# cpuimage/minSDTF

Hardware: AMD Instinct MI355X
Metric: 512x512 images/sec (whole node), SD1.5 25-step txt2img (higher is better)
Workload: dtype bf16; 1 GPU; SD1.5 512x512 25-step txt2img, CFG 7.5 + rescale 0.7, batch 1/GPU, UNet+VAE HIP path, random-init weights; global_batch=1, parallelism=batch-shard x1, hipgraph=True, cond_uncond=one fused batch

## Files before the change

minsdtf_amd/csrc/capi.hip:

```cpp
#include <stdarg.h>
#include <string.h>
#include "common.h"

static thread_local char g_err[512] = "";

void msd_set_error(const char* fmt, ...) {
    va_list ap;
    va_start(ap, fmt);
    vsnprintf(g_err, sizeof(g_err), fmt, ap);
    va_end(ap);
}

int msd_conv_gemm_init();
int msd_attention_init();

extern "C" int msd_abi_version(void) { return MSD_ABI_VERSION; }
extern "C" const char* msd_last_error(void) { return g_err; }
extern "C" int msd_init(void) {
    int rc = msd_conv_gemm_init();
    if (rc) return rc;
    return msd_attention_init();
}

void msd_set_gn_impl(int v);
void msd_set_conv_dense(int v);
void msd_set_gn_rows_q(int v);
void msd_set_gn_wide(int v);
void msd_set_gn_cluster(int v);
void msd_set_gn_rows(int v);
void msd_set_gn_xmap(int v);
void msd_set_gn_poll_limit(int v);
void msd_set_attn_qf(int v);
void msd_set_attn_qf4_min(int v);
void msd_set_xattn_nw(int v);
int msd_set_xattn160_mode(int v);
void msd_set_attn_form(int v);
void msd_set_attn_d160_pipe(int v);
extern "C" int msd_set_option(const char* key, int value) {
    if (key && strcmp(key, "gn_rows_q") == 0) {
        if (value < -1 || value > 2) MSD_FAIL(MSD_E_ARG, "set_option: gn_rows_q %d (-1 .. 2)", value);
        msd_set_gn_rows_q(value);
        return MSD_OK;
    }
    if (key && strcmp(key, "conv_dense") == 0) {
        msd_set_conv_dense(value);
        return MSD_OK;
    }
    if (key && strcmp(key, "attn_qf") == 0) {
        if (value < 0 || value > 4 || value == 3) MSD_FAIL(MSD_E_ARG, "set_option: attn_qf takes 0, 1, 2 or 4");
        msd_set_attn_qf(value);
        return MSD_OK;
    }
    if (key && strcmp(key, "attn_qf4_min") == 0) {
        if (value < 128) MSD_FAIL(MSD_E_ARG, "set_option: attn_qf4_min takes a workgroup count >= 128");
        msd_set_attn_qf4_min(value);
        return MSD_OK;
    }
    if (key && strcmp(key, "attn_form") == 0) {
        if (value < 0 || value > 2) MSD_FAIL(MSD_E_ARG, "set_option: attn_form takes 0, 1 or 2");
        msd_set_attn_form(value);
        return MSD_OK;
    }
    if (key && strcmp(key, "attn_d160_pipe") == 0) {
        msd_set_attn_d160_pipe(value ? 1 : 0);
        return MSD_OK;
    }
    if (key && strcmp(key, "xattn160_mode") == 0) {
        if (!msd_set_xattn160_mode(value)) MSD_FAIL(MSD_E_ARG, "set_option: xattn160_mode %d exists in the instrumented build (make stamps) only", value);
        return MSD_OK;
    }
    if (key && strcmp(key, "xattn_nw") == 0) {
        if (value != 0 && value != 4 && value != 8) MSD_FAIL(MSD_E_ARG, "set_option: xattn_nw takes 0, 4 or 8");
        msd_set_xattn_nw(value);
        return MSD_OK;
    }
    if (key && strcmp(key, "gn_wide") == 0) {
        msd_set_gn_wide(value);
        return MSD_OK;
    }
    if (key && strcmp(key, "gn_xmap") == 0) { msd_set_gn_xmap(value); return MSD_OK; }
    if (key && strcmp(key, "gn_rows") == 0) {
        if (value < 0) MSD_FAIL(MSD_E_ARG, "set_option: gn_rows takes a pixel count >= 0, got %d", value);
        msd_set_gn_rows(value);
        return MSD_OK;
    }
    if (key && strcmp(key, "gn_cluster") == 0) {
        if (value != 0 && (value < 64 || value > (1 << 20))) MSD_FAIL(MSD_E_ARG, "set_option: gn_cluster takes 0 or 64 .. 2^20 pixels per part");
        msd_set_gn_cluster(value);
        return MSD_OK;
    }
    if (key && strcmp(key, "gn_poll_limit") == 0) {
        if (value < 1) MSD_FAIL(MSD_E_ARG, "set_option: gn_poll_limit takes a positive count");
        msd_set_gn_poll_limit(value);
        return MSD_OK;
    }
    if (key && strcmp(key, "gn_impl") == 0) {
        msd_set_gn_impl(value);
        return MSD_OK;
    }
    MSD_FAIL(MSD_E_ARG, "set_option: unknown key");
}
```

minsdtf_amd/csrc/conv_rowpanel.hip:

```cpp
#include "conv_common.h"

constexpr int RL_STEPS = 4;
template <int KC, int MI, bool RL = false>
__global__ __launch_bounds__(256) void dense_rowpanel_kernel(const bf16_t* hot_a0, const bf16_t* hot_w, int hot_M, int hot_N, int hot_c0, int hot_tiles_m, int hot_tiles_n,
                                                             uint32_t hot_w_rs, uint32_t hot_w_ks, int wg_cols, int nsplits, uint32_t mg_nsplits, const CGArgs p) {
    constexpr int S = 3, NJ = 2, MP = MI / 2;
    constexpr int BM = 4 * MI * 16;
    constexpr int W_BYTES = KC * 4096;
    static_assert(MI % 2 == 0, "row fragments pair up for the 16-byte stores");
    extern __shared__ __attribute__((aligned(16))) char smem[];
    const uint32_t lds0 = (uint32_t)(size_t)(__attribute__((address_space(3))) char*)smem;
    float* l_bias = reinterpret_cast<float*>(smem + S * W_BYTES);
    float* l_cs = l_bias + wg_cols;

    const int tid = threadIdx.x, lane = tid & 63;
    const int wave = __builtin_amdgcn_readfirstlane(tid >> 6);
    const int r = lane & 15, g = lane >> 4;
    const int tile = xcd_remap(blockIdx.x, hot_tiles_m * hot_tiles_n);
    const int panel = udiv_magic(tile, nsplits, mg_nsplits), ns = tile - panel * nsplits;
    const int m0 = panel * BM + wave * (MI * 16);
    const int n0 = ns * wg_cols;
    const int nsteps = (min(wg_cols, hot_N - n0)) >> 5;

    const int cpos = tid & 7, lrow = tid >> 3;
    const uint32_t wsw = (uint32_t)((cpos ^ ((lrow >> 1) & 7)) * 16);
    const uint32_t lds_wave = lds0 + (uint32_t)(wave * 8) * 128u;
    auto issue_w = [&](int step, int stage) {
        const uint32_t off = (uint32_t)min(n0 + step * 32 + lrow, hot_N - 1) * hot_w_rs + wsw;
        const uint32_t base = __builtin_amdgcn_readfirstlane(lds_wave + (uint32_t)stage * W_BYTES);
#pragma unroll
        for (int kc = 0; kc < KC; ++kc) dma16s(hot_w, off + (uint32_t)kc * hot_w_ks, base + (uint32_t)kc * 4096u);
    };
    if (nsteps > 0) issue_w(0, 0);
    if (nsteps > 1) issue_w(1, 1);

    bf16x8 af[MI][KC * 2];
#pragma unroll
    for (int i = 0; i < MI; ++i) {
        const bf16_t* src = hot_a0 + (size_t)min(m0 + i * 16 + r, hot_M - 1) * hot_c0 + g * 8;
#pragma unroll
        for (int ks = 0; ks < KC * 2; ++ks) af[i][ks] = *reinterpret_cast<const bf16x8*>(src + ks * 32);
    }
    for (int t = tid; t < wg_cols; t += 256) {
        const int n = min(n0 + t, p.N - 1);
        l_bias[t] = p.bias ? p.bias[n] : 0.f;
        l_cs[t] = (!RL && p.ln_in) ? p.ln_colsum[n] : 0.f;
    }
    const int cgo = cg_col(g), cg8 = (g & 1) << 3;
    const int rw = cg_wrow(r);
    int msw[MP], bidx[MI];
#pragma unroll
    for (int ip = 0; ip < MP; ++ip) msw[ip] = m0 + (g < 2 ? 2 * ip : 2 * ip + 1) * 16 + r;
    typedef uint32_t u32x4 __attribute__((ext_vector_type(4)));
    u32x4 rres[RL ? RL_STEPS : 1][MP][NJ];
    if (RL) {
#pragma unroll
        for (int st = 0; st < RL_STEPS; ++st)
#pragma unroll
            for (int ip = 0; ip < MP; ++ip)
#pragma unroll
                for (int j = 0; j < NJ; ++j) {
                    rres[st][ip][j] = (u32x4){0, 0, 0, 0};
                    if (p.residual && st < nsteps)
                        rres[st][ip][j] = *reinterpret_cast<const u32x4*>(p.residual + (size_t)min(msw[ip], p.M - 1) * p.res_ld +
                                                                          min(n0 + st * 32 + j * 16 + cg8, p.N - 8));
                }
    }
    constexpr int LNS = LN_MAX_SLOTS / 4;
    float mean[MI], rstd[MI];
#pragma unroll
    for (int i = 0; i < MI; ++i) { mean[i] = 0.f; rstd[i] = 1.f; }
    if (!RL && p.ln_in) {
        float2 lnp[MI][LNS];
#pragma unroll
        for (int i = 0; i < MI; ++i) {
            const float2* src = reinterpret_cast<const float2*>(p.ln_in) + (size_t)min(m0 + i * 16 + r, p.M - 1) * p.ln_in_slots;
#pragma unroll
            for (int k = 0; k < LNS; ++k) lnp[i][k] = src[min(g + 4 * k, p.ln_in_slots - 1)];
        }
        wait_vmcnt<0>();
#pragma unroll
        for (int i = 0; i < MI; ++i) {
            float s1 = 0.f, s2 = 0.f;
#pragma unroll
            for (int k = 0; k < LNS; ++k)
                if (g + 4 * k < p.ln_in_slots) { s1 += lnp[i][k].x; s2 += lnp[i][k].y; }
            s1 += __shfl_xor(s1, 16); s2 += __shfl_xor(s2, 16);
            s1 += __shfl_xor(s1, 32); s2 += __shfl_xor(s2, 32);
            mean[i] = s1 * p.ln_inv_k;
            rstd[i] = rsqrtf(fmaxf(s2 * p.ln_inv_k - mean[i] * mean[i], 0.f) + p.ln_eps);
        }
    }
    wait_vmcnt<0>();
#pragma unroll
    for (int i = 0; i < MI; ++i)
#pragma unroll
        for (int ks = 0; ks < KC * 2; ++ks) asm volatile("" : "+v"(af[i][ks]));
    if (RL) {
#pragma unroll
        for (int st = 0; st < RL_STEPS; ++st)
#pragma unroll
            for (int ip = 0; ip < MP; ++ip)
#pragma unroll
                for (int j = 0; j < NJ; ++j) asm volatile("" : "+v"(rres[st][ip][j]));
    }
    __syncthreads();

    float lna[MP], lnq[MP];
#pragma unroll
    for (int ip = 0; ip < MP; ++ip) { lna[ip] = 0.f; lnq[ip] = 0.f; }
#pragma unroll
    for (int i = 0; i < MI; ++i) bidx[i] = p.split_mode ? udiv_magic(min(m0 + i * 16 + r, p.M - 1), p.hw_out, p.mg_hw) : 0;
    auto swap8 = [&](const float (&a)[4], const float (&b)[4], float (&v)[8]) {
#pragma unroll
        for (int e = 0; e < 4; ++e) {
            auto sw = __builtin_amdgcn_permlane32_swap(__float_as_uint(a[e]), __float_as_uint(b[e]), false, false);
            v[e] = __uint_as_float(sw[0]);
            v[4 + e] = __uint_as_float(sw[1]);
        }
    };

    int stage = 0;
    for (int step = 0; step < nsteps; ++step) {
        if (step) {
            if (step + 1 < nsteps) wait_vmcnt<KC>();
            else wait_vmcnt<0>();
            __builtin_amdgcn_s_barrier();
        }
        if (step + 2 < nsteps) {
            int st = stage + 2;
            if (st >= S) st -= S;
            issue_w(step + 2, st);
        }
        f32x4 acc[NJ][MI];
#pragma unroll
        for (int j = 0; j < NJ; ++j)
#pragma unroll
            for (int i = 0; i < MI; ++i) acc[j][i] = (f32x4){0.f, 0.f, 0.f, 0.f};
        const char* bW = smem + stage * W_BYTES + rw * 128;
#pragma unroll
        for (int kc = 0; kc < KC; ++kc) {
            bf16x8 wf[2][NJ];
#pragma unroll
            for (int ks = 0; ks < 2; ++ks)
#pragma unroll
                for (int j = 0; j < NJ; ++j)
                    wf[ks][j] = *reinterpret_cast<const bf16x8*>(bW + kc * 4096 + j * 16 * 128 + (((ks * 4 + g) ^ (rw >> 1)) << 4));
#pragma unroll
            for (int ks = 0; ks < 2; ++ks)
#pragma unroll
                for (int j = 0; j < NJ; ++j)
#pragma unroll
                    for (int i = 0; i < MI; ++i)
                        acc[j][i] = __builtin_amdgcn_mfma_f32_16x16x32_bf16(wf[ks][j], af[i][kc * 2 + ks], acc[j][i], 0, 0, 0);
        }
        const int nb = n0 + step * 32;
        float4 bv[NJ], cs[NJ];
#pragma unroll
        for (int j = 0; j < NJ; ++j) {
            bv[j] = *reinterpret_cast<const float4*>(l_bias + step * 32 + j * 16 + cgo);
            cs[j] = *reinterpret_cast<const float4*>(l_cs + step * 32 + j * 16 + cgo);
        }
        if (!RL && p.ln_in) {
#pragma unroll
            for (int i = 0; i < MI; ++i)
#pragma unroll
                for (int j = 0; j < NJ; ++j) {
                    acc[j][i][0] = rstd[i] * (acc[j][i][0] - mean[i] * cs[j].x);
                    acc[j][i][1] = rstd[i] * (acc[j][i][1] - mean[i] * cs[j].y);
                    acc[j][i][2] = rstd[i] * (acc[j][i][2] - mean[i] * cs[j].z);
                    acc[j][i][3] = rstd[i] * (acc[j][i][3] - mean[i] * cs[j].w);
                }
        }
        if constexpr (RL) {
            const float zero = 0.f;
#pragma unroll
            for (int i = 0; i < MI; ++i)
#pragma unroll
                for (int j = 0; j < NJ; ++j) {
                    acc[j][i][0] = (acc[j][i][0] + bv[j].x) + zero; acc[j][i][1] = (acc[j][i][1] + bv[j].y) + zero;
                    acc[j][i][2] = (acc[j][i][2] + bv[j].z) + zero; acc[j][i][3] = (acc[j][i][3] + bv[j].w) + zero;
                }
            if ((step & 1) == 0) {
#pragma unroll
                for (int ip = 0; ip < MP; ++ip) { lna[ip] = 0.f; lnq[ip] = 0.f; }
            }
#pragma unroll
            for (int ip = 0; ip < MP; ++ip)
#pragma unroll
                for (int j = 0; j < NJ; ++j) {
                    float a[4] = {acc[j][2 * ip][0], acc[j][2 * ip][1], acc[j][2 * ip][2], acc[j][2 * ip][3]};
                    float b[4] = {acc[j][2 * ip + 1][0], acc[j][2 * ip + 1][1], acc[j][2 * ip + 1][2], acc[j][2 * ip + 1][3]};
                    float v[8], q[8];
                    swap8(a, b, v);
                    u32x4 rr = rres[0][ip][j];
#pragma unroll
                    for (int st = 1; st < RL_STEPS; ++st) if (step == st) rr = rres[st][ip][j];
                    unpack8(make_uint4(rr.x, rr.y, rr.z, rr.w), q);
#pragma unroll
                    for (int e = 0; e < 8; ++e) v[e] = v[e] + q[e];
                    const uint4 o = pack8(v);
                    const bool ok = msw[ip] < p.M;
                    if (ok) *reinterpret_cast<uint4*>(reinterpret_cast<bf16_t*>(p.out) + (size_t)msw[ip] * p.out_ld + nb + j * 16 + cg8) = o;
                    if (p.ln_out) {
                        unpack8(o, q);
                        float s1 = (ok ? (q[0] + q[1]) + (q[2] + q[3]) : 0.f) + (ok ? (q[4] + q[5]) + (q[6] + q[7]) : 0.f);
                        float s2 = (ok ? (q[0] * q[0] + q[1] * q[1]) + (q[2] * q[2] + q[3] * q[3]) : 0.f) +
                                   (ok ? (q[4] * q[4] + q[5] * q[5]) + (q[6] * q[6] + q[7] * q[7]) : 0.f);
                        auto t1 = __builtin_amdgcn_permlane16_swap(__float_as_uint(s1), __float_as_uint(s1), false, false);
                        auto t2 = __builtin_amdgcn_permlane16_swap(__float_as_uint(s2), __float_as_uint(s2), false, false);
                        lna[ip] += __uint_as_float(t1[0]) + __uint_as_float(t1[1]);
                        lnq[ip] += __uint_as_float(t2[0]) + __uint_as_float(t2[1]);
                    }
                }
            if (p.ln_out && (step & 1) && (g & 1) == 0) {
#pragma unroll
                for (int ip = 0; ip < MP; ++ip)
                    if (msw[ip] < p.M)
                        reinterpret_cast<float2*>(p.ln_out)[(size_t)msw[ip] * p.ln_out_slots + (nb >> 6)] = make_float2(lna[ip], lnq[ip]);
            }
        } else if (p.act == MSD_ACT_GEGLU) {
            auto gl4 = [&](int i, float (&v)[4]) {
                v[0] = geglu_f(acc[0][i][0] + bv[0].x, acc[1][i][0] + bv[1].x);
                v[1] = geglu_f(acc[0][i][1] + bv[0].y, acc[1][i][1] + bv[1].y);
                v[2] = geglu_f(acc[0][i][2] + bv[0].z, acc[1][i][2] + bv[1].z);
                v[3] = geglu_f(acc[0][i][3] + bv[0].w, acc[1][i][3] + bv[1].w);
            };
#pragma unroll
            for (int ip = 0; ip < MP; ++ip) {
                float a[4], b[4], v[8];
                gl4(2 * ip, a);
                gl4(2 * ip + 1, b);
                swap8(a, b, v);
                if (msw[ip] < p.M)
                    *reinterpret_cast<uint4*>(reinterpret_cast<bf16_t*>(p.out) + (size_t)msw[ip] * p.out_ld + (nb >> 1) + cg8) = pack8(v);
            }
        } else {
            const float zero = 0.f;
#pragma unroll
            for (int i = 0; i < MI; ++i)
#pragma unroll
                for (int j = 0; j < NJ; ++j) {
                    acc[j][i][0] = (acc[j][i][0] + bv[j].x) + zero; acc[j][i][1] = (acc[j][i][1] + bv[j].y) + zero;
                    acc[j][i][2] = (acc[j][i][2] + bv[j].z) + zero; acc[j][i][3] = (acc[j][i][3] + bv[j].w) + zero;
                }
#pragma unroll
            for (int j = 0; j < NJ; ++j) {
                const int nbj = nb + j * 16;
                if (p.split_mode == 0 || nbj < p.ns0 + p.ns1) {
#pragma unroll
                    for (int ip = 0; ip < MP; ++ip) {
                        float a[4] = {acc[j][2 * ip][0], acc[j][2 * ip][1], acc[j][2 * ip][2], acc[j][2 * ip][3]};
                        float b[4] = {acc[j][2 * ip + 1][0], acc[j][2 * ip + 1][1], acc[j][2 * ip + 1][2], acc[j][2 * ip + 1][3]};
                        float v[8];
                        swap8(a, b, v);
                        if (p.split_mode == 0) {
#pragma unroll
                            for (int e = 0; e < 8; ++e) v[e] = v[e] + zero;
                        }
                        const int n8 = nbj + cg8;
                        if (msw[ip] >= p.M) continue;
                        bf16_t* dst = (p.split_mode == 0 || n8 < p.ns0) ? reinterpret_cast<bf16_t*>(p.out) + (size_t)msw[ip] * p.out_ld + n8
                                                                         : p.out1 + (size_t)msw[ip] * p.out1_ld + (n8 - p.ns0);
                        *reinterpret_cast<uint4*>(dst) = pack8(v);
                    }
                } else {
                    const int nv = p.N - p.ns0 - p.ns1;
                    const int nn = nbj + cgo - p.ns0 - p.ns1;
#pragma unroll
                    for (int i = 0; i < MI; ++i) {
                        const int m = m0 + i * 16 + r;
                        if (m >= p.M) continue;
                        const int sidx = m - bidx[i] * p.hw_out;
                        const uint32_t ox = pack_bf2(acc[j][i][0], acc[j][i][1]), oy = pack_bf2(acc[j][i][2], acc[j][i][3]);
                        bf16_t* dst = p.out2 + ((size_t)bidx[i] * nv + nn) * p.out2_ld + sidx;
                        dst[0] = (bf16_t)(ox & 0xFFFF);
                        dst[(size_t)p.out2_ld] = (bf16_t)(ox >> 16);
                        dst[(size_t)2 * p.out2_ld] = (bf16_t)(oy & 0xFFFF);
                        dst[(size_t)3 * p.out2_ld] = (bf16_t)(oy >> 16);
                    }
                }
            }
        }
        if (++stage == S) stage = 0;
    }
}

static bool g_rp_attr_done = false;
constexpr int rp_lds(int kc, int wg_cols) { return 3 * kc * 4096 + 2 * wg_cols * 4; }
constexpr int RP_MAX_COLS = 1024;

int msd_conv_rowpanel_init() {
    if (g_rp_attr_done) return MSD_OK;
    hipError_t e = hipFuncSetAttribute(reinterpret_cast<const void*>(&dense_rowpanel_kernel<5, 2>), hipFuncAttributeMaxDynamicSharedMemorySize, rp_lds(5, RP_MAX_COLS));
    if (e == hipSuccess) e = hipFuncSetAttribute(reinterpret_cast<const void*>(&dense_rowpanel_kernel<10, 2>), hipFuncAttributeMaxDynamicSharedMemorySize, rp_lds(10, RP_MAX_COLS));
    if (e == hipSuccess) e = hipFuncSetAttribute(reinterpret_cast<const void*>(&dense_rowpanel_kernel<5, 2, true>), hipFuncAttributeMaxDynamicSharedMemorySize, rp_lds(5, 32 * RL_STEPS));
    if (e == hipSuccess) e = hipFuncSetAttribute(reinterpret_cast<const void*>(&dense_rowpanel_kernel<10, 2, true>), hipFuncAttributeMaxDynamicSharedMemorySize, rp_lds(10, 32 * RL_STEPS));
    if (e != hipSuccess) MSD_FAIL((int)e, "hipFuncSetAttribute(conv_rowpanel): %s", hipGetErrorString(e));
    g_rp_attr_done = true;
    return MSD_OK;
}

bool msd_conv_rowpanel_eligible(const CGArgs& a, int rows, int wg_cols) {
    const bool rl = a.residual || a.ln_out;
    const bool shape = a.ksize == 1 && a.stride == 1 && !a.upsample && a.c1 == 0 && !a.a2 && (a.K == 320 || a.K == 640) && (a.N % 32) == 0 &&
                       !a.rowvec && !a.out_f32 && a.nslices == 1 && a.vec16 &&
                       (a.act == MSD_ACT_NONE || (a.act == MSD_ACT_GEGLU && a.split_mode == 0)) &&
                       (!rl || (a.act == MSD_ACT_NONE && a.split_mode == 0 && !a.ln_in && (a.N % 64) == 0 && (wg_cols % 64) == 0 &&
                                wg_cols <= 32 * RL_STEPS)) &&
                       (long long)a.M * a.c0 * 2 < (1ll << 32) - 4096;
    const bool cfg = rows == 128;
    return shape && cfg && wg_cols >= 32 && wg_cols <= RP_MAX_COLS && (wg_cols % 32) == 0;
}

int msd_conv_rowpanel_launch(CGArgs a, int rows, int wg_cols, hipStream_t stream) {
    int rc = msd_conv_rowpanel_init();
    if (rc) return rc;
    if (wg_cols > a.N) wg_cols = a.N;
    const int panels = (a.M + rows - 1) / rows, nsplits = (a.N + wg_cols - 1) / wg_cols;
    a.tiles_m = panels; a.tiles_n = nsplits;
    const dim3 grid(panels * nsplits);
    const uint32_t mg = udiv_magic_of(nsplits);
    const bool rl = a.residual || a.ln_out;
    if (a.K == 320) {
        if (rl) hipLaunchKernelGGL((dense_rowpanel_kernel<5, 2, true>), grid, dim3(256), rp_lds(5, wg_cols), stream, a.a0, a.w, a.M, a.N, a.c0, a.tiles_m, a.tiles_n, a.w_rs, a.w_ks, wg_cols, nsplits, mg, a);
        else hipLaunchKernelGGL((dense_rowpanel_kernel<5, 2>), grid, dim3(256), rp_lds(5, wg_cols), stream, a.a0, a.w, a.M, a.N, a.c0, a.tiles_m, a.tiles_n, a.w_rs, a.w_ks, wg_cols, nsplits, mg, a);
    } else {
        if (rl) hipLaunchKernelGGL((dense_rowpanel_kernel<10, 2, true>), grid, dim3(256), rp_lds(10, wg_cols), stream, a.a0, a.w, a.M, a.N, a.c0, a.tiles_m, a.tiles_n, a.w_rs, a.w_ks, wg_cols, nsplits, mg, a);
        else hipLaunchKernelGGL((dense_rowpanel_kernel<10, 2>), grid, dim3(256), rp_lds(10, wg_cols), stream, a.a0, a.w, a.M, a.N, a.c0, a.tiles_m, a.tiles_n, a.w_rs, a.w_ks, wg_cols, nsplits, mg, a);
    }
    return MSD_OK;
}
```

Before: 10.39 images/s.

## Software-pipeline K=640 rowpanel GEMM: overlap next tile MFMA with current epilogue

Adds a PIPE variant of the dense rowpanel kernel for K=640 non-residual launches. It double-buffers the accumulators so the MFMA work for the next 32-column step is interleaved with the epilogue of the current step, using sched_group_barrier hints. It also double-buffers the LDS weight fragments across the kc loop and keeps the A fragments in AGPRs. The weight prefetch is moved one step earlier. The variant is on by default and can be switched off through a new rowpanel_pipe option. It risks higher register pressure and a more fragile instruction schedule, and it also adds optional timing-stamp instrumentation under MSD_STAMPS.

```diff
diff --git a/minsdtf_amd/csrc/capi.hip b/minsdtf_amd/csrc/capi.hip
--- a/minsdtf_amd/csrc/capi.hip
+++ b/minsdtf_amd/csrc/capi.hip
@@ -36,6 +36,7 @@
 int msd_set_xattn160_mode(int v);
 void msd_set_attn_form(int v);
 void msd_set_attn_d160_pipe(int v);
+void msd_set_rowpanel_pipe(int v);
 extern "C" int msd_set_option(const char* key, int value) {
     if (key && strcmp(key, "gn_rows_q") == 0) {
         if (value < -1 || value > 2) MSD_FAIL(MSD_E_ARG, "set_option: gn_rows_q %d (-1 .. 2)", value);
@@ -63,6 +64,10 @@
     }
     if (key && strcmp(key, "attn_d160_pipe") == 0) {
         msd_set_attn_d160_pipe(value ? 1 : 0);
+        return MSD_OK;
+    }
+    if (key && strcmp(key, "rowpanel_pipe") == 0) {
+        msd_set_rowpanel_pipe(value ? 1 : 0);
         return MSD_OK;
     }
     if (key && strcmp(key, "xattn160_mode") == 0) {
diff --git a/minsdtf_amd/csrc/conv_rowpanel.hip b/minsdtf_amd/csrc/conv_rowpanel.hip
--- a/minsdtf_amd/csrc/conv_rowpanel.hip
+++ b/minsdtf_amd/csrc/conv_rowpanel.hip
@@ -1,10 +1,65 @@
 #include "conv_common.h"
 
 constexpr int RL_STEPS = 4;
-template <int KC, int MI, bool RL = false>
+
+#ifdef MSD_STAMPS
+extern "C" MSD_API int msd_debug_stamps_rowpanel(unsigned long long* host_out, int count) {
+    return (int)hipMemcpyFromSymbol(host_out, HIP_SYMBOL(g_stamps), sizeof(unsigned long long) * (size_t)count);
+}
+__device__ __forceinline__ unsigned long long rp_now() {
+    unsigned long long t;
+    __builtin_amdgcn_sched_barrier(0);
+    asm volatile("s_memrealtime %0\n\ts_waitcnt lgkmcnt(0)" : "=s"(t)::"memory");
+    __builtin_amdgcn_sched_barrier(0);
+    return t;
+}
+#define RP_STAMP_VARS unsigned long long rp_t = 0, rp_sum[4] = {0, 0, 0, 0}
+#define RP_MARK() rp_t = rp_now()
+#define RP_LAP(i)                                  \
+    do {                                           \
+        const unsigned long long rp_n = rp_now();  \
+        rp_sum[(i) - 8] += rp_n - rp_t;            \
+        rp_t = rp_n;                               \
+    } while (0)
+#define RP_MFMA_RETIRE(x)                                          \
+    do {                                                           \
+        float rp_d;                                                \
+        asm volatile("v_mov_b32 %0, %1" : "=v"(rp_d) : "v"(x));   \
+    } while (0)
+#define RP_STAMP_FLUSH(steps)                                                                                         \
+    do {                                                                                                              \
+        if (threadIdx.x == 0) {                                                                                       \
+            unsigned long long* rp_o = g_stamps + (((size_t)blockIdx.y * gridDim.x + blockIdx.x) & 8191) * 16;        \
+            rp_o[8] = rp_sum[0]; rp_o[9] = rp_sum[1]; rp_o[10] = rp_sum[2]; rp_o[11] = rp_sum[3];                   \
+            rp_o[12] = (unsigned long long)(steps);                                                                   \
+        }                                                                                                             \
+    } while (0)
+#else
+#define RP_STAMP_VARS
+#define RP_MARK()
+#define RP_LAP(i)
+#define RP_MFMA_RETIRE(x)
+#define RP_STAMP_FLUSH(steps)
+#endif
+
+template <int KC>
+__device__ __forceinline__ void rp_interleave() {
+    __builtin_amdgcn_sched_group_barrier(0x100, 4, 0);
+#pragma unroll
+    for (int kc = 0; kc < KC; ++kc) {
+        if (kc + 1 < KC) __builtin_amdgcn_sched_group_barrier(0x100, 4, 0);
+#pragma unroll
+        for (int m = 0; m < 8; ++m) {
+            __builtin_amdgcn_sched_group_barrier(0x8, 1, 0);
+            __builtin_amdgcn_sched_group_barrier(0x2, 3, 0);
+        }
+    }
+}
+template <int KC, int MI, bool RL = false, bool PIPE = false>
 __global__ __launch_bounds__(256) void dense_rowpanel_kernel(const bf16_t* hot_a0, const bf16_t* hot_w, int hot_M, int hot_N, int hot_c0, int hot_tiles_m, int hot_tiles_n,
                                                              uint32_t hot_w_rs, uint32_t hot_w_ks, int wg_cols, int nsplits, uint32_t mg_nsplits, const CGArgs p) {
     constexpr int S = 3, NJ = 2, MP = MI / 2;
+    static_assert(!PIPE || (KC > 5 && !RL), "the pipelined loop exists for K = 640, consumer form");
     constexpr int BM = 4 * MI * 16;
     constexpr int W_BYTES = KC * 4096;
     static_assert(MI % 2 == 0, "row fragments pair up for the 16-byte stores");
@@ -16,6 +71,7 @@
     const int tid = threadIdx.x, lane = tid & 63;
     const int wave = __builtin_amdgcn_readfirstlane(tid >> 6);
     const int r = lane & 15, g = lane >> 4;
+    MSD_STAMP(0);
     const int tile = xcd_remap(blockIdx.x, hot_tiles_m * hot_tiles_n);
     const int panel = udiv_magic(tile, nsplits, mg_nsplits), ns = tile - panel * nsplits;
     const int m0 = panel * BM + wave * (MI * 16);
@@ -95,7 +151,10 @@
 #pragma unroll
     for (int i = 0; i < MI; ++i)
 #pragma unroll
-        for (int ks = 0; ks < KC * 2; ++ks) asm volatile("" : "+v"(af[i][ks]));
+        for (int ks = 0; ks < KC * 2; ++ks) {
+            if constexpr (PIPE) asm volatile("" : "+a"(af[i][ks]));
+            else asm volatile("" : "+v"(af[i][ks]));
+        }
     if (RL) {
 #pragma unroll
         for (int st = 0; st < RL_STEPS; ++st)
@@ -105,6 +164,8 @@
                 for (int j = 0; j < NJ; ++j) asm volatile("" : "+v"(rres[st][ip][j]));
     }
     __syncthreads();
+    MSD_STAMP(1);
+    MSD_STAMP_DRAIN();
 
     float lna[MP], lnq[MP];
 #pragma unroll
@@ -120,40 +181,50 @@
         }
     };
 
-    int stage = 0;
-    for (int step = 0; step < nsteps; ++step) {
-        if (step) {
-            if (step + 1 < nsteps) wait_vmcnt<KC>();
-            else wait_vmcnt<0>();
-            __builtin_amdgcn_s_barrier();
-        }
-        if (step + 2 < nsteps) {
-            int st = stage + 2;
-            if (st >= S) st -= S;
-            issue_w(step + 2, st);
-        }
-        f32x4 acc[NJ][MI];
+    RP_STAMP_VARS;
+    auto mfma_tile = [&](int stage, f32x4 (&acc)[NJ][MI]) {
 #pragma unroll
         for (int j = 0; j < NJ; ++j)
 #pragma unroll
             for (int i = 0; i < MI; ++i) acc[j][i] = (f32x4){0.f, 0.f, 0.f, 0.f};
         const char* bW = smem + stage * W_BYTES + rw * 128;
+        auto frag = [&](int kc, int ks, int j) {
+            return *reinterpret_cast<const bf16x8*>(bW + kc * 4096 + j * 16 * 128 + (((ks * 4 + g) ^ (rw >> 1)) << 4));
+        };
+        bf16x8 wf[PIPE ? 2 : 1][2][NJ];
+        if constexpr (PIPE) {
+#pragma unroll
+            for (int ks = 0; ks < 2; ++ks)
+#pragma unroll
+                for (int j = 0; j < NJ; ++j) wf[0][ks][j] = frag(0, ks, j);
+        }
 #pragma unroll
         for (int kc = 0; kc < KC; ++kc) {
-            bf16x8 wf[2][NJ];
+            const int cur = PIPE ? (kc & 1) : 0;
+            if constexpr (PIPE) {
+                if (kc + 1 < KC) {
+#pragma unroll
+                    for (int ks = 0; ks < 2; ++ks)
+#pragma unroll
+                        for (int j = 0; j < NJ; ++j) wf[cur ^ 1][ks][j] = frag(kc + 1, ks, j);
+                }
+            } else {
+#pragma unroll
+                for (int ks = 0; ks < 2; ++ks)
+#pragma unroll
+                    for (int j = 0; j < NJ; ++j) wf[0][ks][j] = frag(kc, ks, j);
+            }
 #pragma unroll
             for (int ks = 0; ks < 2; ++ks)
 #pragma unroll
                 for (int j = 0; j < NJ; ++j)
-                    wf[ks][j] = *reinterpret_cast<const bf16x8*>(bW + kc * 4096 + j * 16 * 128 + (((ks * 4 + g) ^ (rw >> 1)) << 4));
-#pragma unroll
-            for (int ks = 0; ks < 2; ++ks)
-#pragma unroll
-                for (int j = 0; j < NJ; ++j)
 #pragma unroll
                     for (int i = 0; i < MI; ++i)
-                        acc[j][i] = __builtin_amdgcn_mfma_f32_16x16x32_bf16(wf[ks][j], af[i][kc * 2 + ks], acc[j][i], 0, 0, 0);
-        }
+                        acc[j][i] = __builtin_amdgcn_mfma_f32_16x16x32_bf16(wf[cur][ks][j], af[i][kc * 2 + ks], acc[j][i], 0, 0, 0);
+        }
+    };
+
+    auto epilogue = [&](int step, f32x4 (&acc)[NJ][MI], auto&& under) {
         const int nb = n0 + step * 32;
         float4 bv[NJ], cs[NJ];
 #pragma unroll
@@ -161,7 +232,8 @@
             bv[j] = *reinterpret_cast<const float4*>(l_bias + step * 32 + j * 16 + cgo);
             cs[j] = *reinterpret_cast<const float4*>(l_cs + step * 32 + j * 16 + cgo);
         }
-        if (!RL && p.ln_in) {
+        const bool ln_fold = !RL && p.ln_in;
+        auto fold = [&]() {
 #pragma unroll
             for (int i = 0; i < MI; ++i)
 #pragma unroll
@@ -170,7 +242,11 @@
                     acc[j][i][1] = rstd[i] * (acc[j][i][1] - mean[i] * cs[j].y);
                     acc[j][i][2] = rstd[i] * (acc[j][i][2] - mean[i] * cs[j].z);
                     acc[j][i][3] = rstd[i] * (acc[j][i][3] - mean[i] * cs[j].w);
-                }
+                    if constexpr (PIPE) asm("" : "+v"(acc[j][i][0]), "+v"(acc[j][i][1]), "+v"(acc[j][i][2]), "+v"(acc[j][i][3]));
+                }
+        };
+        if constexpr (!PIPE) {
+            if (ln_fold) fold();
         }
         if constexpr (RL) {
             const float zero = 0.f;
@@ -226,16 +302,28 @@
                 v[2] = geglu_f(acc[0][i][2] + bv[0].z, acc[1][i][2] + bv[1].z);
                 v[3] = geglu_f(acc[0][i][3] + bv[0].w, acc[1][i][3] + bv[1].w);
             };
+            if constexpr (PIPE) {
+                under();
+                fold();
+            }
+            uint4 o[MP];
 #pragma unroll
             for (int ip = 0; ip < MP; ++ip) {
                 float a[4], b[4], v[8];
                 gl4(2 * ip, a);
                 gl4(2 * ip + 1, b);
                 swap8(a, b, v);
-                if (msw[ip] < p.M)
-                    *reinterpret_cast<uint4*>(reinterpret_cast<bf16_t*>(p.out) + (size_t)msw[ip] * p.out_ld + (nb >> 1) + cg8) = pack8(v);
-            }
+                o[ip] = pack8(v);
+            }
+            if constexpr (PIPE) rp_interleave<KC>();
+#pragma unroll
+            for (int ip = 0; ip < MP; ++ip)
+                if (msw[ip] < p.M) *reinterpret_cast<uint4*>(reinterpret_cast<bf16_t*>(p.out) + (size_t)msw[ip] * p.out_ld + (nb >> 1) + cg8) = o[ip];
         } else {
+            if constexpr (PIPE) {
+                under();
+                fold();
+            }
             const float zero = 0.f;
 #pragma unroll
             for (int i = 0; i < MI; ++i)
@@ -282,20 +370,86 @@
                 }
             }
         }
-        if (++stage == S) stage = 0;
-    }
+    };
+    auto nothing = []() {};
+
+    if constexpr (!PIPE) {
+        int stage = 0;
+        for (int step = 0; step < nsteps; ++step) {
+            RP_MARK();
+            if (step) {
+                if (step + 1 < nsteps) wait_vmcnt<KC>();
+                else wait_vmcnt<0>();
+                RP_LAP(8);
+                __builtin_amdgcn_s_barrier();
+                RP_LAP(9);
+            }
+            if (step + 2 < nsteps) {
+                int st = stage + 2;
+                if (st >= S) st -= S;
+                issue_w(step + 2, st);
+            }
+            f32x4 acc[NJ][MI];
+            mfma_tile(stage, acc);
+            RP_MFMA_RETIRE(acc[NJ - 1][MI - 1][0]);
+            RP_LAP(10);
+            epilogue(step, acc, nothing);
+            RP_LAP(11);
+            if (++stage == S) stage = 0;
+        }
+    } else if (nsteps > 0) {
+        f32x4 accA[NJ][MI], accB[NJ][MI];
+        if (nsteps > 2) issue_w(2, 2);
+        mfma_tile(0, accA);
+        int step = 0, stage = 0;
+        auto top = [&]() {
+            RP_MARK();
+            if (step) {
+                if (step + 2 < nsteps) wait_vmcnt<KC>();
+                else wait_vmcnt<0>();
+            }
+            RP_LAP(8);
+            __builtin_amdgcn_s_barrier();
+            RP_LAP(9);
+            if (step + 3 < nsteps) issue_w(step + 3, stage);
+            if (++stage == S) stage = 0;
+        };
+        while (true) {
+            if (step + 1 >= nsteps) { RP_MARK(); epilogue(step, accA, nothing); RP_LAP(11); break; }
+            top();
+            epilogue(step, accA, [&]() { mfma_tile(stage, accB); });
+            RP_LAP(10);
+            ++step;
+            if (step + 1 >= nsteps) { RP_MARK(); epilogue(step, accB, nothing); RP_LAP(11); break; }
+            top();
+            epilogue(step, accB, [&]() { mfma_tile(stage, accA); });
+            RP_LAP(10);
+            ++step;
+        }
+    }
+    RP_STAMP_FLUSH(nsteps);
+    MSD_STAMP_DRAIN();
+    MSD_STAMP(4);
 }
 
 static bool g_rp_attr_done = false;
 constexpr int rp_lds(int kc, int wg_cols) { return 3 * kc * 4096 + 2 * wg_cols * 4; }
 constexpr int RP_MAX_COLS = 1024;
 
+static int g_rp_pipe = 1;
+void msd_set_rowpanel_pipe(int v) { g_rp_pipe = v; }
+
+template <int KC, bool RL, bool PIPE>
+static hipError_t rp_set_lds(int wg_cols) {
+    return hipFuncSetAttribute(reinterpret_cast<const void*>(&dense_rowpanel_kernel<KC, 2, RL, PIPE>), hipFuncAttributeMaxDynamicSharedMemorySize, rp_lds(KC, wg_cols));
+}
 int msd_conv_rowpanel_init() {
     if (g_rp_attr_done) return MSD_OK;
-    hipError_t e = hipFuncSetAttribute(reinterpret_cast<const void*>(&dense_rowpanel_kernel<5, 2>), hipFuncAttributeMaxDynamicSharedMemorySize, rp_lds(5, RP_MAX_COLS));
-    if (e == hipSuccess) e = hipFuncSetAttribute(reinterpret_cast<const void*>(&dense_rowpanel_kernel<10, 2>), hipFuncAttributeMaxDynamicSharedMemorySize, rp_lds(10, RP_MAX_COLS));
-    if (e == hipSuccess) e = hipFuncSetAttribute(reinterpret_cast<const void*>(&dense_rowpanel_kernel<5, 2, true>), hipFuncAttributeMaxDynamicSharedMemorySize, rp_lds(5, 32 * RL_STEPS));
-    if (e == hipSuccess) e = hipFuncSetAttribute(reinterpret_cast<const void*>(&dense_rowpanel_kernel<10, 2, true>), hipFuncAttributeMaxDynamicSharedMemorySize, rp_lds(10, 32 * RL_STEPS));
+    hipError_t e = rp_set_lds<5, false, false>(RP_MAX_COLS);
+    if (e == hipSuccess) e = rp_set_lds<10, false, false>(RP_MAX_COLS);
+    if (e == hipSuccess) e = rp_set_lds<10, false, true>(RP_MAX_COLS);
+    if (e == hipSuccess) e = rp_set_lds<5, true, false>(32 * RL_STEPS);
+    if (e == hipSuccess) e = rp_set_lds<10, true, false>(32 * RL_STEPS);
     if (e != hipSuccess) MSD_FAIL((int)e, "hipFuncSetAttribute(conv_rowpanel): %s", hipGetErrorString(e));
     g_rp_attr_done = true;
     return MSD_OK;
@@ -322,12 +476,17 @@
     const dim3 grid(panels * nsplits);
     const uint32_t mg = udiv_magic_of(nsplits);
     const bool rl = a.residual || a.ln_out;
+#define RP_LAUNCH(KC, RL, PIPE)                                                                                                            \
+    hipLaunchKernelGGL((dense_rowpanel_kernel<KC, 2, RL, PIPE>), grid, dim3(256), rp_lds(KC, wg_cols), stream, a.a0, a.w, a.M, a.N, a.c0, \
+                       a.tiles_m, a.tiles_n, a.w_rs, a.w_ks, wg_cols, nsplits, mg, a)
     if (a.K == 320) {
-        if (rl) hipLaunchKernelGGL((dense_rowpanel_kernel<5, 2, true>), grid, dim3(256), rp_lds(5, wg_cols), stream, a.a0, a.w, a.M, a.N, a.c0, a.tiles_m, a.tiles_n, a.w_rs, a.w_ks, wg_cols, nsplits, mg, a);
-        else hipLaunchKernelGGL((dense_rowpanel_kernel<5, 2>), grid, dim3(256), rp_lds(5, wg_cols), stream, a.a0, a.w, a.M, a.N, a.c0, a.tiles_m, a.tiles_n, a.w_rs, a.w_ks, wg_cols, nsplits, mg, a);
+        if (rl) RP_LAUNCH(5, true, false);
+        else RP_LAUNCH(5, false, false);
     } else {
-        if (rl) hipLaunchKernelGGL((dense_rowpanel_kernel<10, 2, true>), grid, dim3(256), rp_lds(10, wg_cols), stream, a.a0, a.w, a.M, a.N, a.c0, a.tiles_m, a.tiles_n, a.w_rs, a.w_ks, wg_cols, nsplits, mg, a);
-        else hipLaunchKernelGGL((dense_rowpanel_kernel<10, 2>), grid, dim3(256), rp_lds(10, wg_cols), stream, a.a0, a.w, a.M, a.N, a.c0, a.tiles_m, a.tiles_n, a.w_rs, a.w_ks, wg_cols, nsplits, mg, a);
-    }
+        if (rl) RP_LAUNCH(10, true, false);
+        else if (g_rp_pipe) RP_LAUNCH(10, false, true);
+        else RP_LAUNCH(10, false, false);
+    }
+#undef RP_LAUNCH
     return MSD_OK;
 }
```

Result: no change. 10.42 images/s (median of 3 runs) (+0.3%).
